# jperezrua/mfas

Hardware: AMD Instinct MI355X
Metric: candidate-archs trained/sec (NTU inner loop) (higher is better)
Workload: dtype f32

## Files before the change

### mfas_amd/csrc/launches.hip.h

```cpp
#pragma once
#include <stdint.h>
#include <vector>

struct Launch {
    int sweep_g = -1, upd = 0, fwd = 0;
    int64_t sweep_t = 0;
    int chain_g = -1;
    int64_t chain_t = 0;
    int gather_g = -1, gather_n = 0;
    int64_t gather_b = 0;
};

static void epoch_launches(int ngroups, bool same_group, int64_t T, bool gather, std::vector<Launch>& out) {
    out.clear();
    gather = gather && ngroups == 2;
    auto add = [&](int gs, int upd, int fwd, int64_t ts, int gc, int64_t tc) -> Launch& {
        out.push_back(Launch{gs, upd, fwd, ts, gc, tc});
        return out.back();
    };
    auto rows = [&](Launch& l, int g, int64_t b, int n) { if (gather) { l.gather_g = g; l.gather_b = b; l.gather_n = n; } };
    for (int g = 0; g < ngroups; ++g) rows(add(g, 0, 1, 0, -1, 0), g, 0, T > 1 ? 2 : 1);
    if (ngroups == 1 && same_group) {
        for (int64_t t = 0; t < T; ++t) add(0, 1, t + 1 < T, t, 0, t);
    } else if (ngroups == 1) {
        for (int64_t t = 0; t < T; ++t) { add(-1, 0, 0, 0, 0, t); add(0, 1, t + 1 < T, t, -1, 0); }
    } else {
        add(-1, 0, 0, 0, 0, 0);
        for (int64_t t = 0; t < T; ++t) {
            const int fwd = t + 1 < T;
            Launch& a = add(0, 1, fwd, t, 1, t);
            if (t >= 1 && t + 1 < T) rows(a, 1, t + 1, 1);
            Launch& b = add(1, 1, fwd, t, fwd ? 0 : -1, t + 1);
            if (fwd && t + 2 < T) rows(b, 0, t + 2, 1);
        }
    }
}
```

### mfas_amd/csrc/mfas_hip.hip

```cpp
#include <hip/hip_runtime.h>
#include <hip/hip_fp16.h>
#pragma clang fp contract(off)
#include <stdint.h>
#include <stdio.h>
#include <string.h>
#include <math.h>
#include <algorithm>
#include <string>
#include <vector>
#include <thread>
#include <chrono>
#include <dlfcn.h>

#include "mfas_hip.h"

#include "common.hip.h"
#include "sweep.hip.h"
#include "chain.hip.h"

struct StepArgs {
    SweepArgs sa;
    ChainArgs ca;
    int32_t nchain, _pad;
    GatherArgs ga;
};

template <int MB, bool NT, int WPE, bool LEAN, int NS = 1>
__global__ void __launch_bounds__(STEP_THREADS, WPE) k_step(const StepArgs a) {
    extern __shared__ __attribute__((aligned(16))) float lds[];
    const int bid = (int)blockIdx.x;
    if (bid < a.nchain) {
        if constexpr (NS > 1) {
            const int Kp = a.nchain / NS, part = bid / Kp, c = bid - part * Kp;
            if (c < a.ca.ncand) chain_split<NS>(a.ca, chain_step_of(a.ca), c, part, lds);
        } else
        if constexpr (LEAN) { chain_lean<MB, 0, (WPE >= 4 ? 8 : 16)>(a.ca, chain_step_of(a.ca), bid, lds, lean_pre<MB>(a.ca, bid)); chain_lean_tail<MB, 0>(a.ca, chain_step_of(a.ca), bid, lds); }
        else chain_body<MB, false>(a.ca, chain_step_of(a.ca), bid, lds);
    }
    else if (bid < a.nchain + a.ga.nblocks) gather_body(a.ga, a.ga.cands[bid - a.nchain], a.sa.g, a.sa.tab, a.sa.order, (int)threadIdx.x);
    else if (bid < a.nchain + a.ga.nblocks + a.sa.ntap) sweep_tap_body<MB, NT, SweepU<MB, WPE>::v>(a.sa, bid - a.nchain - a.ga.nblocks, lds);
    else sweep_body<MB, NT, SweepU<MB, WPE>::v>(a.sa, sweep_step_of(a.sa), bid - a.nchain - a.ga.nblocks - a.sa.ntap, lds);
}

template <int MB, bool NT, int NS = 1>
__global__ void __launch_bounds__(STEP_THREADS, 4) k_step_same(const StepArgs a) {
    extern __shared__ __attribute__((aligned(16))) float lds[];
    const int bid = (int)blockIdx.x;
    if (bid < a.nchain) {
        if constexpr (NS > 1) {
            const int Kp = a.nchain / NS, part = bid / Kp, c = bid - part * Kp;
            if (c < a.ca.ncand) chain_split<NS>(a.ca, chain_step_of(a.ca), c, part, lds);
        } else chain_body<MB, false, true>(a.ca, chain_step_of(a.ca), bid, lds);
    } else sweep_body<MB, NT, SweepU<MB, 4>::v, true>(a.sa, sweep_step_of(a.sa), bid - a.nchain, lds);
}

template <int MB, bool LEAN>
__global__ void __launch_bounds__(STEP_THREADS, 2) k_chain(const ChainArgs a) {
    extern __shared__ __attribute__((aligned(16))) float lds[];
    if constexpr (LEAN) { chain_lean<MB>(a, chain_step_of(a), (int)blockIdx.x, lds, lean_pre<MB>(a, (int)blockIdx.x)); chain_lean_tail<MB, 0>(a, chain_step_of(a), (int)blockIdx.x, lds); }
    else chain_body<MB, true>(a, chain_step_of(a), (int)blockIdx.x, lds);
}

#include "wide.hip.h"
#include "persist.hip.h"
#include "eval.hip.h"
#include "pack.hip.h"

#include "builds.hip.h"
#include "plan.hip.h"

struct LaunchRecord {
    struct Entry { BuildKey key; const void* fn; int64_t n; };
    std::vector<Entry> entries;
    void clear() { entries.clear(); }
// ... 552 lines not shown
```

### mfas_amd/csrc/plan.hip.h

```cpp
#pragma once
struct Tuning {
    int persist = -1;
    int no_lean_chain = 0;
    int groups = 0;
    int same_group = -1;
    int no_tap_major = 0;
    int force_tap_major = 0;
    int no_red_in_sweep = 0;
    double occ_bytes = -1.0;
    int no_xcd_placement = 0;
    int n_xcd = 0;
    int persist_trace = 0;
    int nt = -1;
    int eval_no_x16 = 0;
    int eval_no_msplit = 0;
    int eval_no_b3 = 0;
    int eval_no_wl = 0;
    int no_gather = 0;
    int gather_verbose = 0;
    int no_plain_chain = 0;
    int persist_verbose = 0;
    int prof_every = 16;
    int chain_split = -1;
    int test_not_resident = -1;
// ... 96 lines not shown

static Geo make_geo(const mfas_hyper* hp) {
    Geo g;
    memset(&g, 0, sizeof(g));
    g.R = hp->R; g.C = hp->C; g.Rp = ceil16(hp->R); g.Cp = ceil16(hp->C);
    g.nrb = g.Rp / 16; g.ncb = g.Cp / 16; g.B = hp->B;
    g.MB = (hp->B + 15) / 16; if (g.MB == 3) g.MB = 4;
    g.Bp = g.MB * 16;
    g.bn = hp->bn != 0; g.alphas = hp->alphas != 0; g.multitask = hp->multitask != 0;
    g.use_drop = hp->drpt > 1e-10;
    g.drop_scale = g.use_drop ? (float)(1.0 / (1.0 - hp->drpt)) : 1.0f;
    g.drop_thr = g.use_drop ? (uint32_t)floor(hp->drpt * 16777216.0) : 0u;
    g.bn_eps = (float)hp->bn_eps; g.bn_mom = (float)hp->bn_momentum;
    g.vec_cell_stride = 5 * g.Rp + 16;
    g.vec_head = MFAS_MAX_CELLS * g.vec_cell_stride;
    for (int j = 0; j < MFAS_MAX_TAPS; ++j) { g.sw[j] = ceil16(hp->s_sizes[j]); g.vw[j] = ceil16(hp->v_sizes[j]); }
    g.loss_mode = hp->loss_mode == 1 ? 1 : 0;
    g.f1_th = (float)hp->f1_threshold;
    return g;
}

static size_t res_batch_lds(const mfas_hyper* hp, const Geo& g, int cc) {
    return hp->tap_bits == 16 ? (size_t)g.Bp * (cc + 8) * 2 : (size_t)g.Bp * (cc + 4) * 4;
}
static size_t res_unit_lds(const mfas_hyper* hp, const Geo& g, int cc, int nu) {
    return (size_t)nu * 2 * res_batch_lds(hp, g, cc) + (size_t)STEP_NW * g.MB * 256 * 4 + 4 * PERSIST_LDS_WORDS + 64;
}
static size_t sweep_unit_lds(const Geo& g, const SegDesc& d) {
    const int nrb = d.rows_p / 16;
    size_t fl = (size_t)g.Bp * (d.cc + 16) + (size_t)g.Bp * (d.cc + 4) + (size_t)g.Bp * (d.rows_p + 16);
    if (nrb < STEP_NW && d.kind <= KIND_V) fl += (size_t)STEP_NW * nrb * g.MB * 256;
    return fl * 4;
}
static size_t wide_unit_lds(const SegDesc& d) {
    return wide_sweep_lds_floats(std::min(16 * WIDE_KB, d.cc), std::min(16 * WIDE_RBG, d.rows_p)) * 4;
}
static size_t wide_chain_lds(const Geo& g) { return wide_chain_lds_floats(g.Rp, g.Cp, g.Bp) * 4; }
static size_t vec_lds(const Geo& g) { return (size_t)3 * (MFAS_MAX_CELLS * g.vec_cell_stride + g.Cp) * 4; }
static size_t lean_chain_lds(const Geo& g) {
    return ((size_t)2 * MFAS_MAX_CELLS * g.Bp * 20 + (size_t)g.Bp * (g.Cp + 4) + MFAS_MAX_CELLS * 16 + 3 * g.Bp + 16
            + (size_t)(g.alphas ? 2 : 1) * MFAS_MAX_CELLS * g.MB * 256 + vec_lds(g) / 4 + LEAN_SCR + 8 + LeanLds<1>::stage_floats() + (size_t)g.Bp * 64) * 4;
}

struct ChunkPlan {
    bool want_persist = false;
    int target = 0, nu = 1;
    bool plan_res = false;
    int nfeat = 0, max_fcc = 0;
    bool res_ok = false, res_wide = false, lean_ok = false;
    int nres_wg = 0;
    bool resident = false;
};

static ChunkPlan plan_chunk(const mfas_hyper* hp, const Geo& g, const int32_t* confs, const int32_t* n_cells, int K, int chunk_cols,
                            int n_cus, bool allow_persist, const Tuning& tu) {
    ChunkPlan lp;
    lp.want_persist = allow_persist && tu.persist != 0;
    lp.lean_ok = g.nrb == 1 && g.ncb <= 4 && g.MB <= 2 && lean_chain_lds(g) <= 78 * 1024 && !tu.no_lean_chain;
    lp.plan_res = lp.want_persist && g.nrb == 1 && g.MB <= 2 && lp.lean_ok;
    auto feat_units = [&](int cc_target, int* max_cc) {
        int64_t n = 0;
        int mx = 0;
        for (int k = 0; k < K; ++k)
            for (int i = 0; i < n_cells[k] && i < MFAS_MAX_CELLS; ++i) {
                const int sw = ceil16(hp->s_sizes[confs[(k * 4 + i) * 3] & 7]), vw = ceil16(hp->v_sizes[confs[(k * 4 + i) * 3 + 1] & 7]);
                const int cs = pick_chunk(sw, cc_target), cv = pick_chunk(vw, cc_target);
// ... 49 lines not shown
}

struct GroupPlan {
    int c0 = 0, nc = 0;
    double alg_state = 0, alg_feat = 0;
    std::vector<SegDesc> descs;
    std::vector<TapDesc> taps;
};

struct LayoutPlan {
    Geo g;
    int chunk = 0;
    std::vector<CandDev> cands;
    std::vector<SegDesc> descs;
    std::vector<int> desc_start;
    std::vector<int64_t> nparams;
    std::vector<int64_t> cand_plane_base, cand_plane_size;
    int64_t plane_stride = 0, wt_size = 0, step_total = 0;
    double bytes_per_launch = 0.0;
    bool persist = false;
    bool res_chain = false;
    bool res_wide = false;
    int nres = 0;
    int res_nu = 1;
    int nres_wg = 0;
    int res_buf_words = 0;
    bool wide = false;
    std::vector<int> wide_start;
    bool lean_chain = false;
    bool same_group = false;
    int chain_split = 0;
    bool red_in_sweep = false;
    bool nontemporal = false;
    double occ_bytes = 0;
    int mbe = 4, nrbw = 1;
    bool yf_in_lds = false, vec_in_lds = false;
    size_t lds_step = 0, lds_chain = 0, lds_eval = 0;
    bool fits_lds = false;
    size_t lds_split = 0;
    size_t lds_president = 0;
    std::vector<GroupPlan> groups;
    std::vector<SegDesc> pdescs;
    std::vector<int32_t> need;
    std::vector<int32_t> role;
};

static int plan_layout_as(const mfas_hyper* hp, const int32_t* confs, const int32_t* n_cells, const uint32_t* drop_seeds, int K, int chunk_cols,
                          int n_cus, bool allow_persist, const Tuning& tu, const bool wide, LayoutPlan& pl) {
    pl = LayoutPlan();
    pl.wide = wide;
    Geo& g = pl.g;
    g = make_geo(hp);
    const int vec_size = (g.vec_head + g.Cp + 63) & ~63;

    ChunkPlan lp;
    if (wide) {
        lp.target = chunk_cols > 0 ? std::min(16 * WIDE_KB, chunk_cols) : 16 * WIDE_KB;
        lp.target = std::max(16, (lp.target / 16) * 16);
    } else {
        lp = plan_chunk(hp, g, confs, n_cells, K, chunk_cols, n_cus, allow_persist, tu);
        if (lp.res_ok && !lp.resident)
            lp = plan_chunk(hp, g, confs, n_cells, K, chunk_cols, n_cus, false, tu);
    }
    const int target = pl.chunk = lp.target;
    pl.cands.resize(K);
    pl.desc_start.assign(K + 1, 0);
// ... 285 lines not shown
            std::vector<int> prim(nwg), sec(nwg, -1);
            for (int w = 0; w < nwg; ++w) {
                prim[w] = res_cand[w];
                if (pl.res_nu == 2 && w + nwg < (int)res_cand.size()) sec[w] = res_cand[w + nwg];
            }
            for (int c = 0; c < K; ++c) {
                bool any = false;
                for (int w = 0; w < nwg; ++w) any = any || prim[w] == c;
                if (!any) continue;
                const int x = roomiest();
                if (!slots[x].empty()) { take(x, c); chain_xcd[c] = x; }
                for (int w = 0; w < nwg; ++w)
                    if (prim[w] == c && !wg_done[w] && !slots[x].empty()) { take(x, K + w); wg_done[w] = 1; }
            }
            std::vector<int> wg_xcd(nwg, -1);
            for (int b = 0; b < G; ++b) if (role[b] >= K) wg_xcd[role[b] - K] = b % NX;
            for (int c = 0; c < K; ++c) {
                if (chain_xcd[c] >= 0) continue;
                std::vector<int> votes(NX, 0);
                for (int w = 0; w < nwg; ++w) if ((prim[w] == c || sec[w] == c) && wg_xcd[w] >= 0) votes[wg_xcd[w]]++;
                int bx = -1;
                for (int x = 0; x < NX; ++x) if (!slots[x].empty() && (bx < 0 || votes[x] > votes[bx])) bx = x;
                if (bx >= 0) { take(bx, c); chain_xcd[c] = bx; }
            }
            for (int w = 0; w < nwg; ++w)
                if (!wg_done[w]) { const int x = roomiest(); take(x, K + w); wg_done[w] = 1; }
            bool ok = true;
            for (int b = 0; b < G; ++b) ok = ok && role[b] >= 0;
            if (ok) pl.role = role;
        }
    }
    pl.nontemporal = (double)pl.plane_stride * 12.0 > 200.0 * 1024 * 1024;
    if (tu.nt >= 0) pl.nontemporal = tu.nt != 0;
    return MFAS_OK;
}

static int plan_layout(const mfas_hyper* hp, const int32_t* confs, const int32_t* n_cells, const uint32_t* drop_seeds, int K, int chunk_cols,
                       int n_cus, bool allow_persist, const Tuning& tu, LayoutPlan& pl) {
    if (!batch_resident_refuses(hp)) {
        if (int rc = plan_layout_as(hp, confs, n_cells, drop_seeds, K, chunk_cols, n_cus, allow_persist, tu, false, pl)) return rc;
        if (pl.fits_lds) return MFAS_OK;
    }
    return plan_layout_as(hp, confs, n_cells, drop_seeds, K, chunk_cols, n_cus, allow_persist, tu, true, pl);
}

static PlanFacts plan_facts(const LayoutPlan& pl) {
    PlanFacts f;
    f.wide = pl.wide; f.MB = pl.g.MB; f.lean_chain = pl.lean_chain; f.same_group = pl.same_group; f.chain_split = pl.chain_split;
    f.ngroups = (int)pl.groups.size(); f.nontemporal = pl.nontemporal; f.persist = pl.persist; f.res_wide = pl.res_wide; f.res_nu = pl.res_nu;
    f.mbe = pl.mbe; f.nrbw = pl.nrbw; f.nrb = pl.g.nrb;
    return f;
}
```

### mfas_amd/csrc/sweep.hip.h

```cpp
#pragma once
template <int MB, bool NT, int SWEEP_U, bool COH = false>
__device__ __forceinline__ void tile_run(float* Wp, float* Mp, float* Vp, const int rb, const int nkb, const int kb0,
                                         const int kbs, const float* xt, const int ST, const float* xn, const int SN,
                                         const float (&dyf)[MB * 4], const float gsc, const AdamC& ac, const bool upd,
                                         const bool fwd, f32x4 (&yacc)[MB], float* T, const int tstride_rb,
                                         const int lane, const int nj) {
    const int l15 = lane & 15, lg = lane >> 4;
    const float a_ss = ac.ss, a_bc2s = ac.bc2s, a_w1 = ac.w1, a_b2 = ac.b2, a_w2 = ac.w2, a_eps = ac.eps, a_wd = ac.wd;
    for (int kbb = kb0; kbb < nkb; kbb += SWEEP_U * kbs) {
        f32x4 w4[SWEEP_U], m4[SWEEP_U], v4[SWEEP_U];
#pragma unroll
        for (int u = 0; u < SWEEP_U; ++u) {
            const int kb = kbb + u * kbs;
            if (kb < nkb) {
                const int64_t off = ((int64_t)rb * nkb + kb) * 256 + lane * 4;
                w4[u] = NT ? __builtin_nontemporal_load(reinterpret_cast<const f32x4*>(Wp + off))
                           : *reinterpret_cast<const f32x4*>(Wp + off);
                if (upd) {
                    m4[u] = NT ? __builtin_nontemporal_load(reinterpret_cast<const f32x4*>(Mp + off))
                               : *reinterpret_cast<const f32x4*>(Mp + off);
                    v4[u] = NT ? __builtin_nontemporal_load(reinterpret_cast<const f32x4*>(Vp + off))
                               : *reinterpret_cast<const f32x4*>(Vp + off);
                }
            }
        }
#pragma unroll
        for (int u = 0; u < SWEEP_U; ++u) {
            const int kb = kbb + u * kbs;
            if (kb < nkb) {
                const int64_t off = ((int64_t)rb * nkb + kb) * 256 + lane * 4;
                if (upd) {
                    f32x4 acc = {0.f, 0.f, 0.f, 0.f};
                    DW_BATCH_LOOP(MB, (COH ? MB * 4 : nj), acc = MFMA16(xt[(4 * j + lg) * ST + kb * 16 + l15], dyf[j], acc))
                    { f32x4 w = w4[u], m = m4[u], v = v4[u];
                      adam4(w, m, v, acc * gsc, a_ss, a_bc2s, a_w1, a_b2, a_w2, a_eps, a_wd);
                      w4[u] = w; m4[u] = m; v4[u] = v; }
                    if (NT) {
                        __builtin_nontemporal_store(w4[u], reinterpret_cast<f32x4*>(Wp + off));
                        __builtin_nontemporal_store(m4[u], reinterpret_cast<f32x4*>(Mp + off));
                        __builtin_nontemporal_store(v4[u], reinterpret_cast<f32x4*>(Vp + off));
                    } else {
                        *reinterpret_cast<f32x4*>(Wp + off) = w4[u];
                        *reinterpret_cast<f32x4*>(Mp + off) = m4[u];
                        *reinterpret_cast<f32x4*>(Vp + off) = v4[u];
                    }
                    if (T) {
                        float* Tt = T + ((int64_t)kb * tstride_rb + rb) * 256;
                        const int base = (((l15 >> 2) * 16 + 4 * lg) << 2) + (l15 & 3);
#pragma unroll
                        for (int q = 0; q < 4; ++q) Tt[base + 4 * q] = w4[u][q];
                    }
                }
                if (fwd) {
#pragma unroll
                    for (int mb = 0; mb < MB; ++mb) {
                        const f32x4 x4 = *reinterpret_cast<const f32x4*>(xn + (mb * 16 + l15) * SN + kb * 16 + 4 * lg);
#pragma unroll
                        for (int q = 0; q < 4; ++q) yacc[mb] = MFMA16(x4[q], w4[u][q], yacc[mb]);
                    }
                }
            }
        }
    }
}

#define STEP_NW 8
#define STEP_THREADS (STEP_NW * 64)

struct SweepArgs {
    const SegDesc* desc;
    const TapDesc* tdesc;
    int32_t ntap, _padt;
    const CandDev* cands;
    float* plane;
    int64_t plane_stride;
    float* wt;
    float* stepbuf;
    mfas_table tab;
    const int32_t* order;
    int64_t pos_t, pos_n;
    int32_t base_t, base_n, nvalid_t, nvalid_n;
    int32_t do_update, do_forward;
    AdamC ac;
    Geo g;
    uint32_t* red_cnt;
    const uint32_t* cellflag;
    uint32_t flag_target;
    int32_t* flag_status;
    const char* gather;
    int64_t g_cand_stride, g_par_stride;
    int32_t g_par_t, g_par_n;
};

__device__ __forceinline__ int64_t gather_tap_off(const Geo& g, const int kind, const int tap, const int eb) {
    int64_t o = 0;
#pragma unroll
    for (int u = 0; u < MFAS_MAX_TAPS; ++u) {
        if (kind == KIND_V || u < tap) o += g.sw[u];
        if (kind == KIND_V && u < tap) o += g.vw[u];
    }
    return o * g.Bp * eb;
}

struct GatherArgs {
    const CandDev* cands;
    char* buf;
    int64_t cand_stride, par_stride;
    int64_t pos[2];
    int32_t base[2], nvalid[2], par[2];
    int32_t nsets, nblocks;
};

__device__ __forceinline__ void gather_body(const GatherArgs& ga, const CandDev& cd, const Geo& g, const mfas_table& tab,
                                            const int32_t* order, const int tid) {
    const int eb = tab.dtype == MFAS_DT_F32 ? 4 : 2;
    const int32_t* ordp = cand_order(order, g, cd.gidx);
    uint32_t used = 0;
    for (int i = 0; i < cd.L; ++i) used |= (1u << cd.conf[i][0]) | (1u << (MFAS_MAX_TAPS + cd.conf[i][1]));
#pragma unroll
    for (int s = 0; s < 2; ++s) {
        if (s >= ga.nsets) break;
        char* dst0 = ga.buf + (int64_t)cd.gidx * ga.cand_stride + (int64_t)ga.par[s] * ga.par_stride;
        for (int kt = 0; kt < 2 * MFAS_MAX_TAPS; ++kt) {
            if (!((used >> kt) & 1u)) continue;
// ... 19 lines not shown
                    if (e < nvec) {
                        const int b = e / vpr, c = e - b * vpr;
                        *reinterpret_cast<u32x4*>(dst + ((int64_t)b * w) * eb + ((int64_t)c << 4)) = v[u];
                    }
                }
            }
        }
    }
}

struct SweepStep {
    int64_t pos_t, pos_n;
    int32_t base_t, base_n, nvalid_t, nvalid_n;
    int32_t upd, fwd;
    float ss, bc2s;
};
__device__ __forceinline__ SweepStep sweep_step_of(const SweepArgs& a) {
    SweepStep s;
    s.pos_t = a.pos_t; s.pos_n = a.pos_n; s.base_t = a.base_t; s.base_n = a.base_n;
    s.nvalid_t = a.nvalid_t; s.nvalid_n = a.nvalid_n; s.upd = a.do_update; s.fwd = a.do_forward;
    s.ss = a.ac.ss; s.bc2s = a.ac.bc2s;
    return s;
}


#ifdef MFAS_CHAIN_TIMING
#define SW_UNIT_STAMP(k) do { if (COH && a.cellflag && a.flag_target == 16u && threadIdx.x == 0 && d.cell == 0 && d.kind == KIND_S && d.k0 == 0 && d.cand == 0) a.flag_status[64 + 29 + (k)] = (int32_t)wall_clock64(); } while (0)
#define SW_END_STAMP() do { if (COH && a.cellflag && a.flag_target == 16u && threadIdx.x == 0) { atomicMax(reinterpret_cast<uint32_t*>(&a.flag_status[64 + 27]), (uint32_t)wall_clock64()); \
        atomicMax(reinterpret_cast<uint32_t*>(&a.flag_status[128 + d.cell * 4 + d.kind]), (uint32_t)wall_clock64()); } } while (0)
#else
#define SW_END_STAMP() do { } while (0)
#define SW_UNIT_STAMP(k) do { } while (0)
#endif
template <int MB, bool NT, int U, bool COH = false>
__device__ __forceinline__ void sweep_body(const SweepArgs& a, const SweepStep& st, const int bid, float* lds) {
    const SegDesc d = a.desc[bid];
    const CandDev& cd = a.cands[d.cand];
    const int tid = threadIdx.x, lane = tid & 63, wave = tid >> 6;
    const int l15 = lane & 15, lg = lane >> 4;
    constexpr int Bp = MB * 16;
    const int cc = d.cc, rows_p = d.rows_p, nrb = rows_p >> 4, nkb = cc >> 4;
    const int ST = cc + 16;
    const int SN = cc + 4;
    const int SD = rows_p + 16;
    float* xt = lds;
    float* xn = xt + Bp * ST;
    float* dyl = xn + Bp * SN;
    float* wred = dyl + Bp * SD;
    const bool feat = d.kind <= KIND_V;
    const bool upd = st.upd != 0;
    const bool fwd = (st.fwd != 0) && feat;
    if (!upd && !fwd) return;
    const int64_t sbo = cd.step_off;
    const bool red = a.red_cnt != nullptr;

    if (!COH && a.gather && feat) {
        const char* gb = a.gather + (int64_t)cd.gidx * a.g_cand_stride + gather_tap_off(a.g, d.kind, d.tap, a.tab.dtype == MFAS_DT_F32 ? 4 : 2);
        if (upd) stage_table(xt, ST, gb + (int64_t)a.g_par_t * a.g_par_stride, a.tab.dtype, d.width, d.k0, cc, nullptr, 0, 0, st.nvalid_t, Bp, tid, STEP_THREADS);
        if (fwd) stage_table(xn, SN, gb + (int64_t)a.g_par_n * a.g_par_stride, a.tab.dtype, d.width, d.k0, cc, nullptr, 0, 0, st.nvalid_n, Bp, tid, STEP_THREADS);
    } else {
    if (upd && feat) {
        const void* tp = d.kind == KIND_S ? a.tab.s[d.tap] : a.tab.v[d.tap];
        stage_table(xt, ST, tp, a.tab.dtype, d.width, d.k0, cc, cand_order(a.order, a.g, cd.gidx), st.pos_t, st.base_t, st.nvalid_t, Bp, tid, STEP_THREADS);
    }
    if (fwd) {
        const void* tp = d.kind == KIND_S ? a.tab.s[d.tap] : a.tab.v[d.tap];
        stage_table(xn, SN, tp, a.tab.dtype, d.width, d.k0, cc, cand_order(a.order, a.g, cd.gidx), st.pos_n, st.base_n, st.nvalid_n, Bp, tid, STEP_THREADS);
    }
    }
    if constexpr (COH) {
        if (upd && a.cellflag) {
            __shared__ int s_go;
            if (tid == 0) {
                const int slot = d.kind == KIND_HEAD ? cd.L - 1 : (d.kind == KIND_OUT ? d.cell - 1 : d.cell);
                const uint32_t* f = a.cellflag + (size_t)cd.gidx * CELLFLAG_STRIDE + slot;
                uint32_t spins = 0;
                int go = 1;
                while (ld_u32_relaxed(f) < a.flag_target) {
                    __builtin_amdgcn_s_sleep(2);
                    if (++spins > CELLFLAG_SPIN_LIMIT) { go = 0; atomicMax(&a.flag_status[cd.gidx], 2); break; }
                }
                s_go = go;
#ifdef MFAS_CHAIN_TIMING
                if (a.flag_target == 16u && slot == 0 && d.kind <= KIND_V) atomicMin(reinterpret_cast<uint32_t*>(&a.flag_status[64 + 28]), (uint32_t)wall_clock64());
#endif
            }
            __syncthreads();
            if (!s_go) return;
            SW_UNIT_STAMP(0);
        }
    }
    if (upd) {
        if (!feat) {
            const int xcell = d.kind == KIND_OUT ? d.cell - 1 : cd.L - 1;
            stage_f32<COH>(xt, ST, a.stepbuf, sbo + a.g.sb_xo + (int64_t)xcell * Bp * a.g.Rp + d.k0, a.g.Rp, cc, Bp, tid, STEP_THREADS);
        }
        const int64_t dsrc = d.kind == KIND_HEAD ? sbo + a.g.sb_dlog : sbo + a.g.sb_dy + (int64_t)d.cell * Bp * a.g.Rp;
        stage_f32<COH>(dyl, SD, a.stepbuf, dsrc + d.rb0 * 16, d.seg_nrb * 16, rows_p, Bp, tid, STEP_THREADS);
    }
    __syncthreads();
    SW_UNIT_STAMP(1);

    float* Wp = a.plane + d.w_off;
    float* Mp = Wp + a.plane_stride;
    float* Vp = Mp + a.plane_stride;
    const AdamC ac = adam_consts(a.ac, upd ? st.ss : 0.f, upd ? st.bc2s : 1.f);
    float gsc = 1.0f;
    if (a.g.alphas && feat && upd) gsc = ldc1<COH>(a.stepbuf + sbo + a.g.sb_gsc + d.cell * 2 + d.kind);

    const bool split_k = nrb < STEP_NW;
    const int rb0 = split_k ? 0 : wave, rbs = split_k ? 1 : STEP_NW;
    const int kb0 = split_k ? wave : 0, kbs = split_k ? STEP_NW : 1;
    const int64_t part = sbo + a.g.sb_part + (((int64_t)(cd.part_cell_off[d.cell] + d.part_idx) * d.seg_nrb * MB) << 8) +
                         (((int64_t)d.rb0 * MB) << 8);

    for (int rb = rb0; rb < nrb; rb += rbs) {
        float dyf[MB * 4];
#pragma unroll
        for (int j = 0; j < MB * 4; ++j) dyf[j] = upd ? dyl[(4 * j + lg) * SD + rb * 16 + l15] : 0.f;
        f32x4 yacc[MB];
#pragma unroll
        for (int mb = 0; mb < MB; ++mb) yacc[mb] = (f32x4){0.f, 0.f, 0.f, 0.f};
        tile_run<MB, NT, U, COH>(Wp, Mp, Vp, rb, nkb, kb0, kbs, xt, ST, xn, SN, dyf, gsc, ac, upd, fwd, yacc,
                                 d.wt_off >= 0 ? a.wt + d.wt_off + ((int64_t)(d.k0 >> 4) * d.seg_nrb + d.rb0) * 256 : nullptr, d.seg_nrb, lane, (a.g.B + 3) >> 2);
        if (fwd) {
#pragma unroll
            for (int mb = 0; mb < MB; ++mb) {
                if (split_k)
                    *reinterpret_cast<f32x4*>(wred + (((wave * nrb + rb) * MB + mb) << 8) + lane * 4) = yacc[mb];
                else if (red) stc4<true>(a.stepbuf, part + ((rb * MB + mb) << 8) + lane * 4, yacc[mb]);
                else
                    stc4<COH>(a.stepbuf, part + ((rb * MB + mb) << 8) + lane * 4, yacc[mb]);
            }
        }
    }
    SW_UNIT_STAMP(2);
    if (!fwd) { SW_END_STAMP(); return; }
    if (split_k) {
        __syncthreads();
        for (int e = tid; e < nrb * MB * 64; e += STEP_THREADS) {
            const int slot = e >> 6, ln = e & 63;
            f32x4 s = *reinterpret_cast<const f32x4*>(wred + (slot << 8) + ln * 4);
#pragma unroll
            for (int w = 1; w < STEP_NW; ++w)
                s += *reinterpret_cast<const f32x4*>(wred + ((w * nrb * MB + slot) << 8) + ln * 4);
            if (red) stc4<true>(a.stepbuf, part + (slot << 8) + ln * 4, s);
            else stc4<COH>(a.stepbuf, part + (slot << 8) + ln * 4, s);
        }
    }
    if (!red) { SW_END_STAMP(); return; }
    asm volatile("s_waitcnt vmcnt(0)" ::: "memory");
    __syncthreads();
    SW_UNIT_STAMP(3);
    int* flagw = reinterpret_cast<int*>(lds);
    const int ns_c = cd.nch_s[d.cell], nch_c = ns_c + cd.nch_v[d.cell];
    if (tid == 0) {
        uint32_t* cnt = a.red_cnt + d.cand * MFAS_MAX_CELLS + d.cell;
        const uint32_t old = __hip_atomic_fetch_add(cnt, 1u, __ATOMIC_RELAXED, __HIP_MEMORY_SCOPE_AGENT);
        const int last = old == (uint32_t)(nch_c - 1);
        if (last) __hip_atomic_store(cnt, 0u, __ATOMIC_RELAXED, __HIP_MEMORY_SCOPE_AGENT);
        flagw[0] = last;
    }
    __syncthreads();
    SW_UNIT_STAMP(4);
    if (!flagw[0]) { SW_END_STAMP(); return; }
    {
        const int snrb = d.seg_nrb;
        const int per_cell = snrb * MB * 64;
        const int64_t part0 = sbo + a.g.sb_part + (((int64_t)cd.part_cell_off[d.cell] * snrb * MB) << 8);
        const int64_t yf0 = sbo + a.g.sb_yf + (int64_t)d.cell * per_cell * 4;
        const int64_t vplane = (int64_t)MFAS_MAX_CELLS * snrb * MB * 256;
        for (int it = tid; it < per_cell; it += STEP_THREADS) {
            f32x4 accS = {0.f, 0.f, 0.f, 0.f}, accV = {0.f, 0.f, 0.f, 0.f};
            constexpr int PB = 8;
            for (int ch0 = 0; ch0 < nch_c; ch0 += PB) {
                f32x4 p8[PB];
#pragma unroll
                for (int u = 0; u < PB; ++u)
// ... 66 lines not shown
```

### mfas_amd/csrc/train.hip.h

```cpp
#pragma once
struct TrainCall {
    mfas_population* p = nullptr;
    const mfas_table *train = nullptr, *dev = nullptr;
    const int32_t* order = nullptr; const float* step_scalars = nullptr;
    int epochs = 0, first = 0, last = 0, B = 0;
    bool segment = false, resume = false, do_dev = false, snapshot_best = false;
    int64_t max_steps = -1, N = 0, nb = 0;
    AdamC ac; StepArgs st;
    std::vector<Launch> launches;
    int64_t launches_T = -1;
    int64_t split_launches[2] = {0, 0};
    size_t ev_used = 0;
    std::vector<double> ev_bytes; int64_t nlaunch = 0;
    bool use_gather = false;
    int64_t g_par_stride = 0, g_cand_stride = 0;
    std::vector<uint32_t> aborts;
    std::vector<double> best_acc;
    double metric_scale = 1.0; std::vector<DevStats> hstats;
    int elt() const { return train->dtype == MFAS_DT_F32 ? 4 : 2; }
    double dev_metric(int k, int ep) const { return (double)hstats[(size_t)k * epochs + ep].dev_corr * metric_scale / (double)dev->N; }
};

static void base_args(mfas_population* p, const mfas_table& tab, const int32_t* order, const Geo& g, const AdamC& ac, SweepArgs& sa, ChainArgs& ca) {
    const LayoutPlan& pl = p->plan;
    sa.cands = p->d_cands; sa.plane = p->plane; sa.plane_stride = pl.plane_stride; sa.wt = p->wt;
    sa.stepbuf = p->stepbuf; sa.tab = tab; sa.order = order; sa.g = g; sa.ac = ac;
    ca.plane = p->plane; ca.plane_stride = pl.plane_stride; ca.wt = p->wt; ca.stepbuf = p->stepbuf;
    ca.tab = tab; ca.order = order; ca.g = g; ca.status = p->d_status; ca.ac = ac;
    ca.yf_in_lds = pl.yf_in_lds ? 1 : 0; ca.vec_in_lds = pl.vec_in_lds ? 1 : 0; ca.pos_w = p->d_posw;
}

static hipError_t setup_gather(TrainCall& c) {
    mfas_population* p = c.p;
    const Geo& g = c.st.sa.g;
    c.use_gather = p->plan.groups.size() == 2 && !p->plan.persist && c.order && g.order_stride > 0 && !p->tune.no_gather;
    if (!c.use_gather) return hipSuccess;
    int64_t totw = 0;
    for (int u = 0; u < MFAS_MAX_TAPS; ++u) totw += g.sw[u] + g.vw[u];
    c.g_par_stride = totw * g.Bp * c.elt(); c.g_cand_stride = 2 * c.g_par_stride;
    const size_t need = (size_t)c.g_cand_stride * p->K;
    if (p->gather_cap < need) {
        hipFree(p->d_gather); p->d_gather = nullptr; p->gather_cap = 0;
        hipError_t e = hipMalloc(&p->d_gather, need);
        if (e != hipSuccess) { c.use_gather = false; (void)hipGetLastError(); return hipSuccess; }
        p->gather_cap = need;
    }
    if (p->tune.gather_verbose) fprintf(stderr, "[gather] on: %d candidates, %.1f MB of gathered rows\n", p->K, (double)need / 1e6);
    return hipSuccess;
}

static hipError_t init_args(TrainCall& c, int64_t ep) {
    mfas_population* p = c.p; StepArgs& st = c.st;
    const LayoutPlan& pl = p->plan; const int K = p->K;
    c.launches_T = -1;
    Geo g = pl.g;
    g.order_stride = (p->hp.order_per_candidate && c.order) ? (int64_t)c.epochs * c.N : 0;
    memset(&st, 0, sizeof(st));
    base_args(p, *c.train, c.order, g, c.ac, st.sa, st.ca);
    st.ca.E = c.epochs; st.ca.stats = p->d_stats;
    st.sa.red_cnt = pl.red_in_sweep ? p->d_red_cnt : nullptr; st.ca.yf_reduced = pl.red_in_sweep ? 1 : 0;
    hipError_t e_ = hipSuccess;
    if (pl.red_in_sweep) e_ = hipMemsetAsync(p->d_red_cnt, 0, sizeof(uint32_t) * K * MFAS_MAX_CELLS, p->stream);
    if (e_ == hipSuccess && pl.same_group) e_ = hipMemsetAsync(p->d_cellflag, 0, sizeof(uint32_t) * K * CELLFLAG_STRIDE, p->stream);
    if (e_ == hipSuccess && pl.chain_split) e_ = hipMemsetAsync(p->d_xch, 0xFF, sizeof(float) * (size_t)K * XCH_CAND_FLOATS, p->stream);
    st.ca.xch = p->d_xch; st.ca.nsplit = pl.chain_split; st.ca.xpar = 0;
    c.split_launches[0] = c.split_launches[1] = 0;
    if (e_ == hipSuccess && ep > 0 && pl.same_group && pl.chain_split)
        e_ = hipMemsetD32Async(reinterpret_cast<hipDeviceptr_t>(p->d_cellflag), (int)((uint32_t)pl.chain_split * (uint32_t)(ep * c.nb)),
                               (size_t)K * CELLFLAG_STRIDE, p->stream);
    return e_ != hipSuccess ? e_ : setup_gather(c);
}

struct ProfBracket {
    TrainCall& c;
    const bool on;
    const double bytes;
    ProfBracket(TrainCall& c_, bool on_, double bytes_) : c(c_), on(on_), bytes(bytes_) {
        if (!on) return;
        mfas_population* p = c.p;
        if (p->ev.size() < c.ev_used + 2) {
            hipEvent_t e0, e1;
            hipEventCreate(&e0); hipEventCreate(&e1); p->ev.push_back(e0); p->ev.push_back(e1);
        }
        hipEventRecord(p->ev[c.ev_used], p->stream);
    }
    ~ProfBracket() {
        if (!on) return;
        hipEventRecord(c.p->ev[c.ev_used + 1], c.p->stream);
        c.ev_used += 2; c.ev_bytes.push_back(bytes);
    }
};

static void launch_record(TrainCall& c, int64_t ep, const Launch& L) {
    mfas_population* p = c.p;
    const LayoutPlan& pl = p->plan;
    StepArgs& st = c.st;
    const int64_t N = c.N;
    const int B = c.B, gs = L.sweep_g, gc = L.chain_g;
    auto nvalid = [&](int64_t t) { return (int)std::min<int64_t>(B, N - t * B); };
    unsigned nsw = 0, nch = 0;
    st.ga.nblocks = 0; st.ga.nsets = 0; st.sa.gather = nullptr;
    if (c.use_gather) {
        GatherArgs& ga = st.ga;
        ga.buf = p->d_gather; ga.cand_stride = c.g_cand_stride; ga.par_stride = c.g_par_stride;
        for (int s = 0; s < L.gather_n; ++s) {
            const int64_t t = L.gather_b + s;
            ga.pos[s] = ep * N + t * B; ga.base[s] = (int)(t * B); ga.nvalid[s] = nvalid(t); ga.par[s] = (int)(t & 1);
        }
        if (L.gather_g >= 0) { ga.nsets = L.gather_n; ga.cands = p->d_cands + pl.groups[L.gather_g].c0; ga.nblocks = pl.groups[L.gather_g].nc; }
        if (gs >= 0 && L.upd) {
            st.sa.gather = p->d_gather; st.sa.g_cand_stride = c.g_cand_stride; st.sa.g_par_stride = c.g_par_stride;
            st.sa.g_par_t = (int)(L.sweep_t & 1); st.sa.g_par_n = (int)((L.sweep_t + 1) & 1);
        }
    }
    if (gs >= 0) {
        SweepArgs& s = st.sa;
        const int64_t ts = L.sweep_t, tn = L.fwd && L.upd ? ts + 1 : ts, gstep = ep * c.nb + ts;
        s.desc = p->groups[gs].d_descs;
        s.tdesc = p->groups[gs].d_taps; s.ntap = (int)pl.groups[gs].taps.size();
        s.do_update = L.upd; s.do_forward = L.fwd;
        s.pos_t = ep * N + ts * B; s.base_t = (int)(ts * B); s.nvalid_t = nvalid(ts);
        s.pos_n = ep * N + tn * B; s.base_n = (int)(tn * B); s.nvalid_n = nvalid(tn);
        s.ac.ss = L.upd ? c.step_scalars[2 * gstep] : 0.f;
        s.ac.bc2s = L.upd ? c.step_scalars[2 * gstep + 1] : 1.f;
        nsw = (unsigned)(pl.groups[gs].descs.size() + pl.groups[gs].taps.size());
    } else st.sa.ntap = 0;
    if (gc >= 0) {
        ChainArgs& ca = st.ca;
        const int64_t tc = L.chain_t, gstep = ep * c.nb + tc;
        ca.cands = p->d_cands + pl.groups[gc].c0;
        ca.pos_t = ep * N + tc * B; ca.base_t = (int)(tc * B); ca.nvalid = nvalid(tc);
        ca.gstep = (int)gstep; ca.epoch = (int)ep;
        ca.ac.ss = c.step_scalars[2 * gstep]; ca.ac.bc2s = c.step_scalars[2 * gstep + 1];
        nch = (unsigned)pl.groups[gc].nc;
    }
    st.nchain = (int)nch;
    if (nsw == 0) {
        launch_build(p, chain_build(chain_key(plan_facts(pl))), nch, pl.lds_chain, p->stream, st.ca);
        return;
    }
    ProfBracket prof(c, p->profiling && L.upd && L.fwd && ((c.nlaunch++ % p->prof_every) == 0),
                     pl.groups[gs].alg_state + pl.groups[gs].alg_feat * c.elt() + 8.0 * B * pl.groups[gs].nc);
    const bool same = pl.same_group && gc == gs && L.upd, split = pl.chain_split && nch > 0;
    if (split) {
        st.ca.ncand = (int)nch; st.ca.xpar = (int)(c.split_launches[gc & 1]++ & 1);
        st.nchain = pl.chain_split * (int)((nch + 7) & ~7u);
    }
    if (same) {
        st.sa.cellflag = p->d_cellflag; st.ca.cellflag = p->d_cellflag;
        st.sa.flag_target = st.ca.flag_target = (split ? (uint32_t)pl.chain_split : 1u) * ((uint32_t)st.ca.gstep + 1u);
        st.sa.flag_status = p->d_status;
    }
    const BuildKey key = step_key(plan_facts(pl), nch, same, pl.groups[gs].alg_state > pl.occ_bytes);
    launch_build(p, step_build(key), (unsigned)st.nchain + st.ga.nblocks + nsw, split ? pl.lds_split : pl.lds_step, p->stream, st);
    if (same) { st.sa.cellflag = nullptr; st.ca.cellflag = nullptr; }
}

static hipError_t persist_epoch_once(TrainCall& c, int ep, int64_t T) {
    mfas_population* p = c.p;
    const LayoutPlan& pl = p->plan;
    const Geo& g = pl.g;
    const int K = p->K;
    if (p->tune.test_not_resident >= 0 && ep >= p->tune.test_not_resident) { c.aborts[ep] = PERSIST_ABORT_NOT_RESIDENT; return hipSuccess; }
    hipError_t e = hipMemsetAsync(p->d_sync, 0, sizeof(uint32_t) * ((size_t)K * PERSIST_SYNC_STRIDE + 64), p->stream);
    if (e != hipSuccess) return e;
    PersistArgs pa;
    memset(&pa, 0, sizeof(pa));
    pa.sa = c.st.sa; pa.ca = c.st.ca;
    pa.sa.desc = p->d_pdescs; pa.sa.tdesc = nullptr; pa.sa.ntap = 0;
    pa.ca.cands = p->d_cands;
    pa.nchain = K; pa.nitems = (int)pl.pdescs.size(); pa.nres = pl.nres; pa.res_chain = pl.res_chain ? 1 : 0; pa.res_wide = pl.res_wide ? 1 : 0;
    pa.res_nu = pl.res_nu; pa.nres_wg = pl.nres_wg; pa.res_buf_words = pl.res_buf_words;
    pa.T = (int)T; pa.epoch = ep;
    pa.lose_step = p->tune.test_lose_step;
// ... 137 lines not shown
    c.ac.eps = (float)hp.adam_eps; c.ac.wd = (float)hp.wd; c.ac.ss = 0.f; c.ac.bc2s = 1.f;
    c.aborts.assign(epochs, 0u);
    HIPCHK(init_args(c, c.first));
    p->prof_launches = 0; p->prof_ms = 0.0; p->prof_bytes = 0.0;
    if (p->plan.persist) {
        const int64_t steps = (int64_t)epochs * c.nb;
        if (p->scal_cap < (size_t)steps * 2) {
            hipFree(p->d_scal); p->d_scal = nullptr;
            HIPCHK(hipMalloc(&p->d_scal, sizeof(float) * steps * 2));
            p->scal_cap = (size_t)steps * 2;
        }
        const size_t have = (size_t)(c.max_steps >= 0 ? std::min<int64_t>(c.max_steps, steps) : steps) * 2;
        HIPCHK(hipMemcpyAsync(p->d_scal, c.step_scalars, sizeof(float) * have, hipMemcpyHostToDevice, p->stream));
    }
    return MFAS_OK;
}

static int train_epoch(TrainCall& c, int ep, int64_t T) {
    mfas_population* p = c.p;
    if (p->plan.persist) {
        HIPCHK(persist_epoch(c, ep, T));
        if (c.aborts[ep] == PERSIST_ABORT_NOT_RESIDENT) {
            if (p->tune.persist_verbose) fprintf(stderr, "[persist] epoch %d: the resident grid never became resident; falling back to launch-per-phase\n", ep);
            if (int rc = persist_fallback(p)) return rc;
            HIPCHK(init_args(c, ep));
            c.aborts[ep] = 0;
        } else if (c.aborts[ep]) {
            HIPCHK(hipStreamSynchronize(p->stream));
            return fail(MFAS_EHIP, "persistent step loop: a workgroup timed out waiting for its dependency (abort code 1: the epoch was "
                                   "abandoned half way, this population's parameters are not usable)");
        }
    }
    if (!p->plan.persist) {
        if (c.launches_T != T) { epoch_launches((int)p->plan.groups.size(), p->plan.same_group, T, c.use_gather, c.launches); c.launches_T = T; }
        for (const Launch& L : c.launches) launch_record(c, ep, L);
    }
    HIPCHK(hipGetLastError());
    return MFAS_OK;
}

static int train_dev(TrainCall& c, int ep) {
    mfas_population* p = c.p;
    const int K = p->K;
    EvalArgs ea;
    memset(&ea, 0, sizeof(ea));
    ea.cands = p->d_cands; ea.plane = p->plane; ea.tab = *c.dev; ea.row0 = 0; ea.nrows = c.dev->N;
    ea.cand0 = 0; ea.epoch = ep; ea.E = c.epochs; ea.g = c.st.sa.g; ea.stats = p->d_stats; ea.pos_w = p->d_posw;
    HIPCHK(launch_eval(p, ea, K, p->stream));
    if (!c.snapshot_best) return MFAS_OK;
    HIPCHK(hipMemcpyAsync(c.hstats.data(), p->d_stats, sizeof(DevStats) * K * c.epochs, hipMemcpyDeviceToHost, p->stream));
    HIPCHK(hipStreamSynchronize(p->stream));
    for (int k = 0; k < K; ++k) {
        const double acc = c.dev_metric(k, ep);
        if (acc > c.best_acc[k]) {
            c.best_acc[k] = acc;
            HIPCHK(hipMemcpyAsync(p->best + p->plan.cand_plane_base[k], p->plane + p->plan.cand_plane_base[k],
                                  sizeof(float) * p->plan.cand_plane_size[k], hipMemcpyDeviceToDevice, p->stream));
        }
    }
    return MFAS_OK;
}

static int train_end(TrainCall& c, mfas_epoch_stats* stats, int32_t* status) {
    mfas_population* p = c.p;
    const int K = p->K, epochs = c.epochs;
    if (c.snapshot_best && c.do_dev && c.last == epochs) {
        HIPCHK(hipMemcpyAsync(p->plane, p->best, sizeof(float) * (size_t)p->plan.plane_stride, hipMemcpyDeviceToDevice, p->stream));
// ... 108 lines not shown
```

Measured before the change: 34.09.

## Defer feature-segment W/m/v stores to every second step via paired Adam updates

Pairs consecutive update launches per group. The first (virtual) launch computes Adam in registers but skips writing W/m/v back to memory. The second (double) launch recomputes the previous step's gradient from a retained previous-batch dy area and gathered rows, applies both Adam steps, and stores once. This is meant to halve weight/optimizer-state write traffic for streaming feature segments. In exchange it triples the gather row sets, alternates between two dy areas in the step buffer, enlarges LDS per unit, and redoes the previous step's MFMA work.

```diff
diff --git a/mfas_amd/csrc/launches.hip.h b/mfas_amd/csrc/launches.hip.h
--- a/mfas_amd/csrc/launches.hip.h
+++ b/mfas_amd/csrc/launches.hip.h
@@ -9,6 +9,7 @@
     int64_t chain_t = 0;
     int gather_g = -1, gather_n = 0;
     int64_t gather_b = 0;
+    int mode = 0;
 };
 
 static void epoch_launches(int ngroups, bool same_group, int64_t T, bool gather, std::vector<Launch>& out) {
@@ -35,3 +36,24 @@
         }
     }
 }
+
+enum { LAUNCH_PLAIN = 0, LAUNCH_VIRTUAL = 1, LAUNCH_DOUBLE = 2 };
+
+static inline void mark_deferred(int ngroups, bool same_group, std::vector<Launch>& list) {
+    for (Launch& l : list) l.mode = LAUNCH_PLAIN;
+    if (ngroups != 2 || same_group) return;
+    for (int g = 0; g < 2; ++g) {
+        Launch* open = nullptr;
+        int64_t n = 0;
+        for (Launch& l : list) {
+            if (l.sweep_g != g || !l.upd) continue;
+            if (open) { open->mode = LAUNCH_VIRTUAL; l.mode = LAUNCH_DOUBLE; open = nullptr; }
+            else if (n >= g) open = &l;
+            ++n;
+        }
+    }
+}
+
+static inline int row_sets(bool deferring) { return deferring ? 3 : 2; }
+static inline int row_set_of(int64_t batch, bool deferring) { return (int)(batch % row_sets(deferring)); }
+static inline int dy_area_of(int64_t step, bool deferring) { return deferring ? (int)(step & 1) : 0; }
diff --git a/mfas_amd/csrc/mfas_hip.hip b/mfas_amd/csrc/mfas_hip.hip
--- a/mfas_amd/csrc/mfas_hip.hip
+++ b/mfas_amd/csrc/mfas_hip.hip
@@ -39,7 +39,7 @@
     }
     else if (bid < a.nchain + a.ga.nblocks) gather_body(a.ga, a.ga.cands[bid - a.nchain], a.sa.g, a.sa.tab, a.sa.order, (int)threadIdx.x);
     else if (bid < a.nchain + a.ga.nblocks + a.sa.ntap) sweep_tap_body<MB, NT, SweepU<MB, WPE>::v>(a.sa, bid - a.nchain - a.ga.nblocks, lds);
-    else sweep_body<MB, NT, SweepU<MB, WPE>::v>(a.sa, sweep_step_of(a.sa), bid - a.nchain - a.ga.nblocks - a.sa.ntap, lds);
+    else sweep_body<MB, NT, SweepU<MB, WPE>::v, false, !LEAN>(a.sa, sweep_step_of(a.sa), bid - a.nchain - a.ga.nblocks - a.sa.ntap, lds);
 }
 
 template <int MB, bool NT, int NS = 1>
diff --git a/mfas_amd/csrc/plan.hip.h b/mfas_amd/csrc/plan.hip.h
--- a/mfas_amd/csrc/plan.hip.h
+++ b/mfas_amd/csrc/plan.hip.h
@@ -152,6 +152,13 @@
     if (nrb < STEP_NW && d.kind <= KIND_V) fl += (size_t)STEP_NW * nrb * g.MB * 256;
     return fl * 4;
 }
+static size_t sweep_unit_lds_double(const Geo& g, const SegDesc& d) {
+    const int nrb = d.rows_p / 16;
+    const size_t replay = (size_t)g.Bp * (d.cc + 16) + (size_t)g.Bp * (d.rows_p + 16), slab = (size_t)STEP_NW * g.MB * 256;
+    size_t fl = (size_t)g.Bp * (d.cc + 16) + (size_t)g.Bp * (d.cc + 4) + (size_t)g.Bp * (d.rows_p + 16);
+    fl += nrb < STEP_NW ? (size_t)(nrb - 1) * slab + std::max(slab, replay) : replay;
+    return fl * 4;
+}
 static size_t wide_unit_lds(const SegDesc& d) {
     return wide_sweep_lds_floats(std::min(16 * WIDE_KB, d.cc), std::min(16 * WIDE_RBG, d.rows_p)) * 4;
 }
@@ -267,6 +274,8 @@
     int chain_split = 0;
     bool red_in_sweep = false;
     bool nontemporal = false;
+    bool defer = false;
+    int64_t sb_dy_alt = 0;
     double occ_bytes = 0;
     int mbe = 4, nrbw = 1;
     bool yf_in_lds = false, vec_in_lds = false;
@@ -618,6 +627,18 @@
     }
     pl.nontemporal = (double)pl.plane_stride * 12.0 > 200.0 * 1024 * 1024;
     if (tu.nt >= 0) pl.nontemporal = tu.nt != 0;
+    pl.defer = pl.groups.size() == 2 && !wide && !pl.persist && !pl.same_group && !pl.lean_chain && !g.alphas;
+    for (const GroupPlan& gr : pl.groups) {
+        if (!gr.taps.empty()) pl.defer = false;
+        for (const SegDesc& d : gr.descs)
+            if (d.kind <= KIND_V && sweep_unit_lds_double(g, d) > pl.lds_step) pl.defer = false;
+    }
+    if (pl.defer) {
+        pl.sb_dy_alt = g.sb_size;
+        g.sb_size = (g.sb_size + (int64_t)MFAS_MAX_CELLS * g.Bp * g.Rp + 63) & ~63LL;
+        for (int k = 0; k < K; ++k) pl.cands[k].step_off = (int64_t)k * g.sb_size;
+        pl.step_total = (int64_t)K * g.sb_size;
+    }
     return MFAS_OK;
 }
 
diff --git a/mfas_amd/csrc/sweep.hip.h b/mfas_amd/csrc/sweep.hip.h
--- a/mfas_amd/csrc/sweep.hip.h
+++ b/mfas_amd/csrc/sweep.hip.h
@@ -1,10 +1,14 @@
 #pragma once
-template <int MB, bool NT, int SWEEP_U, bool COH = false>
+#include "launches.hip.h"
+template <int MB, bool NT, int SWEEP_U, bool COH = false, bool DBL = false>
 __device__ __forceinline__ void tile_run(float* Wp, float* Mp, float* Vp, const int rb, const int nkb, const int kb0,
                                          const int kbs, const float* xt, const int ST, const float* xn, const int SN,
                                          const float (&dyf)[MB * 4], const float gsc, const AdamC& ac, const bool upd,
                                          const bool fwd, f32x4 (&yacc)[MB], float* T, const int tstride_rb,
-                                         const int lane, const int nj) {
+                                         const int lane, const int nj, const bool store = true, const float* xp = nullptr,
+                                         const float* dyp = nullptr, const float* dyc = nullptr, const int SDp = 0,
+                                         const float ss_p = 0.f, const float bc2s_p = 1.f) {
+    static_assert(!(DBL && COH), "the same-group launch defers nothing");
     const int l15 = lane & 15, lg = lane >> 4;
     const float a_ss = ac.ss, a_bc2s = ac.bc2s, a_w1 = ac.w1, a_b2 = ac.b2, a_w2 = ac.w2, a_eps = ac.eps, a_wd = ac.wd;
     for (int kbb = kb0; kbb < nkb; kbb += SWEEP_U * kbs) {
@@ -30,12 +34,24 @@
             if (kb < nkb) {
                 const int64_t off = ((int64_t)rb * nkb + kb) * 256 + lane * 4;
                 if (upd) {
+                    int dq = lg * SDp + rb * 16 + l15;
+                    if constexpr (DBL) asm volatile("" : "+v"(dq));
+                    if constexpr (DBL) {
+                        f32x4 accp = {0.f, 0.f, 0.f, 0.f};
+                        DW_BATCH_LOOP(MB, nj, accp = MFMA16(xp[(4 * j + lg) * ST + kb * 16 + l15], dyp[dq + 4 * j * SDp], accp))
+                        f32x4 w = w4[u], m = m4[u], v = v4[u];
+                        adam4(w, m, v, accp * gsc, ss_p, bc2s_p, a_w1, a_b2, a_w2, a_eps, a_wd);
+                        w4[u] = w; m4[u] = m; v4[u] = v;
+                        __builtin_amdgcn_sched_barrier(0);
+                    }
                     f32x4 acc = {0.f, 0.f, 0.f, 0.f};
-                    DW_BATCH_LOOP(MB, (COH ? MB * 4 : nj), acc = MFMA16(xt[(4 * j + lg) * ST + kb * 16 + l15], dyf[j], acc))
+                    if constexpr (DBL) { DW_BATCH_LOOP(MB, nj, acc = MFMA16(xt[(4 * j + lg) * ST + kb * 16 + l15], dyc[dq + 4 * j * SDp], acc)) }
+                    else { DW_BATCH_LOOP(MB, (COH ? MB * 4 : nj), acc = MFMA16(xt[(4 * j + lg) * ST + kb * 16 + l15], dyf[j], acc)) }
                     { f32x4 w = w4[u], m = m4[u], v = v4[u];
                       adam4(w, m, v, acc * gsc, a_ss, a_bc2s, a_w1, a_b2, a_w2, a_eps, a_wd);
                       w4[u] = w; m4[u] = m; v4[u] = v; }
-                    if (NT) {
+                    if (!COH && !DBL && !store) {
+                    } else if (NT) {
                         __builtin_nontemporal_store(w4[u], reinterpret_cast<f32x4*>(Wp + off));
                         __builtin_nontemporal_store(m4[u], reinterpret_cast<f32x4*>(Mp + off));
                         __builtin_nontemporal_store(v4[u], reinterpret_cast<f32x4*>(Vp + off));
@@ -90,6 +106,10 @@
     const char* gather;
     int64_t g_cand_stride, g_par_stride;
     int32_t g_par_t, g_par_n;
+    int32_t mode, g_par_p;
+    int64_t pos_p, sb_dy_prev;
+    int32_t base_p, nvalid_p;
+    float ss_p, bc2s_p;
 };
 
 __device__ __forceinline__ int64_t gather_tap_off(const Geo& g, const int kind, const int tap, const int eb) {
@@ -175,7 +195,7 @@
 #define SW_END_STAMP() do { } while (0)
 #define SW_UNIT_STAMP(k) do { } while (0)
 #endif
-template <int MB, bool NT, int U, bool COH = false>
+template <int MB, bool NT, int U, bool COH = false, bool DEFER = !COH>
 __device__ __forceinline__ void sweep_body(const SweepArgs& a, const SweepStep& st, const int bid, float* lds) {
     const SegDesc d = a.desc[bid];
     const CandDev& cd = a.cands[d.cand];
@@ -189,21 +209,28 @@
     float* xt = lds;
     float* xn = xt + Bp * ST;
     float* dyl = xn + Bp * SN;
-    float* wred = dyl + Bp * SD;
     const bool feat = d.kind <= KIND_V;
     const bool upd = st.upd != 0;
     const bool fwd = (st.fwd != 0) && feat;
     if (!upd && !fwd) return;
+    float* wred = dyl + Bp * SD;
+    const bool split_k = nrb < STEP_NW;
+    const int mode = (DEFER && feat && upd) ? a.mode : LAUNCH_PLAIN;
+    const bool dbl = mode == LAUNCH_DOUBLE;
+    float* xp = wred + (split_k ? (nrb - 1) * STEP_NW * MB * 256 : 0);
+    float* dyp = xp + Bp * ST;
     const int64_t sbo = cd.step_off;
     const bool red = a.red_cnt != nullptr;
 
     if (!COH && a.gather && feat) {
         const char* gb = a.gather + (int64_t)cd.gidx * a.g_cand_stride + gather_tap_off(a.g, d.kind, d.tap, a.tab.dtype == MFAS_DT_F32 ? 4 : 2);
+        if (dbl) stage_table(xp, ST, gb + (int64_t)a.g_par_p * a.g_par_stride, a.tab.dtype, d.width, d.k0, cc, nullptr, 0, 0, a.nvalid_p, Bp, tid, STEP_THREADS);
         if (upd) stage_table(xt, ST, gb + (int64_t)a.g_par_t * a.g_par_stride, a.tab.dtype, d.width, d.k0, cc, nullptr, 0, 0, st.nvalid_t, Bp, tid, STEP_THREADS);
         if (fwd) stage_table(xn, SN, gb + (int64_t)a.g_par_n * a.g_par_stride, a.tab.dtype, d.width, d.k0, cc, nullptr, 0, 0, st.nvalid_n, Bp, tid, STEP_THREADS);
     } else {
     if (upd && feat) {
         const void* tp = d.kind == KIND_S ? a.tab.s[d.tap] : a.tab.v[d.tap];
+        if (dbl) stage_table(xp, ST, tp, a.tab.dtype, d.width, d.k0, cc, cand_order(a.order, a.g, cd.gidx), a.pos_p, a.base_p, a.nvalid_p, Bp, tid, STEP_THREADS);
         stage_table(xt, ST, tp, a.tab.dtype, d.width, d.k0, cc, cand_order(a.order, a.g, cd.gidx), st.pos_t, st.base_t, st.nvalid_t, Bp, tid, STEP_THREADS);
     }
     if (fwd) {
@@ -240,6 +267,7 @@
         }
         const int64_t dsrc = d.kind == KIND_HEAD ? sbo + a.g.sb_dlog : sbo + a.g.sb_dy + (int64_t)d.cell * Bp * a.g.Rp;
         stage_f32<COH>(dyl, SD, a.stepbuf, dsrc + d.rb0 * 16, d.seg_nrb * 16, rows_p, Bp, tid, STEP_THREADS);
+        if (dbl) stage_f32<false>(dyp, SD, a.stepbuf, sbo + a.sb_dy_prev + (int64_t)d.cell * Bp * a.g.Rp + d.rb0 * 16, d.seg_nrb * 16, rows_p, Bp, tid, STEP_THREADS);
     }
     __syncthreads();
     SW_UNIT_STAMP(1);
@@ -251,7 +279,6 @@
     float gsc = 1.0f;
     if (a.g.alphas && feat && upd) gsc = ldc1<COH>(a.stepbuf + sbo + a.g.sb_gsc + d.cell * 2 + d.kind);
 
-    const bool split_k = nrb < STEP_NW;
     const int rb0 = split_k ? 0 : wave, rbs = split_k ? 1 : STEP_NW;
     const int kb0 = split_k ? wave : 0, kbs = split_k ? STEP_NW : 1;
     const int64_t part = sbo + a.g.sb_part + (((int64_t)(cd.part_cell_off[d.cell] + d.part_idx) * d.seg_nrb * MB) << 8) +
@@ -259,18 +286,30 @@
 
     for (int rb = rb0; rb < nrb; rb += rbs) {
         float dyf[MB * 4];
-#pragma unroll
-        for (int j = 0; j < MB * 4; ++j) dyf[j] = upd ? dyl[(4 * j + lg) * SD + rb * 16 + l15] : 0.f;
         f32x4 yacc[MB];
 #pragma unroll
         for (int mb = 0; mb < MB; ++mb) yacc[mb] = (f32x4){0.f, 0.f, 0.f, 0.f};
-        tile_run<MB, NT, U, COH>(Wp, Mp, Vp, rb, nkb, kb0, kbs, xt, ST, xn, SN, dyf, gsc, ac, upd, fwd, yacc,
-                                 d.wt_off >= 0 ? a.wt + d.wt_off + ((int64_t)(d.k0 >> 4) * d.seg_nrb + d.rb0) * 256 : nullptr, d.seg_nrb, lane, (a.g.B + 3) >> 2);
+        float* Tt = d.wt_off >= 0 ? a.wt + d.wt_off + ((int64_t)(d.k0 >> 4) * d.seg_nrb + d.rb0) * 256 : nullptr;
+        bool plain_walk = true;
+        if constexpr (DEFER) {
+            if (dbl) {
+                plain_walk = false;
+                tile_run<MB, NT, (U > 1 ? U / 2 : 1), false, true>(Wp, Mp, Vp, rb, nkb, kb0, kbs, xt, ST, xn, SN, dyf, gsc, ac, upd, fwd, yacc, Tt, d.seg_nrb,
+                                                                    lane, (a.g.B + 3) >> 2, true, xp, dyp, dyl, SD, a.ss_p, a.bc2s_p);
+                if (split_k && fwd && rb == nrb - 1) __syncthreads();
+            }
+        }
+        if (plain_walk) {
+#pragma unroll
+            for (int j = 0; j < MB * 4; ++j) dyf[j] = upd ? dyl[(4 * j + lg) * SD + rb * 16 + l15] : 0.f;
+            tile_run<MB, NT, U, COH>(Wp, Mp, Vp, rb, nkb, kb0, kbs, xt, ST, xn, SN, dyf, gsc, ac, upd, fwd, yacc, Tt, d.seg_nrb, lane,
+                                     (a.g.B + 3) >> 2, mode != LAUNCH_VIRTUAL);
+        }
         if (fwd) {
 #pragma unroll
             for (int mb = 0; mb < MB; ++mb) {
                 if (split_k)
-                    *reinterpret_cast<f32x4*>(wred + (((wave * nrb + rb) * MB + mb) << 8) + lane * 4) = yacc[mb];
+                    *reinterpret_cast<f32x4*>(wred + (((rb * STEP_NW + wave) * MB + mb) << 8) + lane * 4) = yacc[mb];
                 else if (red) stc4<true>(a.stepbuf, part + ((rb * MB + mb) << 8) + lane * 4, yacc[mb]);
                 else
                     stc4<COH>(a.stepbuf, part + ((rb * MB + mb) << 8) + lane * 4, yacc[mb]);
@@ -283,10 +322,11 @@
         __syncthreads();
         for (int e = tid; e < nrb * MB * 64; e += STEP_THREADS) {
             const int slot = e >> 6, ln = e & 63;
-            f32x4 s = *reinterpret_cast<const f32x4*>(wred + (slot << 8) + ln * 4);
+            const int srb = slot / MB, smb = slot - srb * MB;
+            f32x4 s = *reinterpret_cast<const f32x4*>(wred + (((srb * STEP_NW) * MB + smb) << 8) + ln * 4);
 #pragma unroll
             for (int w = 1; w < STEP_NW; ++w)
-                s += *reinterpret_cast<const f32x4*>(wred + ((w * nrb * MB + slot) << 8) + ln * 4);
+                s += *reinterpret_cast<const f32x4*>(wred + (((srb * STEP_NW + w) * MB + smb) << 8) + ln * 4);
             if (red) stc4<true>(a.stepbuf, part + (slot << 8) + ln * 4, s);
             else stc4<COH>(a.stepbuf, part + (slot << 8) + ln * 4, s);
         }
diff --git a/mfas_amd/csrc/train.hip.h b/mfas_amd/csrc/train.hip.h
--- a/mfas_amd/csrc/train.hip.h
+++ b/mfas_amd/csrc/train.hip.h
@@ -37,7 +37,7 @@
     if (!c.use_gather) return hipSuccess;
     int64_t totw = 0;
     for (int u = 0; u < MFAS_MAX_TAPS; ++u) totw += g.sw[u] + g.vw[u];
-    c.g_par_stride = totw * g.Bp * c.elt(); c.g_cand_stride = 2 * c.g_par_stride;
+    c.g_par_stride = totw * g.Bp * c.elt(); c.g_cand_stride = row_sets(p->plan.defer) * c.g_par_stride;
     const size_t need = (size_t)c.g_cand_stride * p->K;
     if (p->gather_cap < need) {
         hipFree(p->d_gather); p->d_gather = nullptr; p->gather_cap = 0;
@@ -45,7 +45,9 @@
         if (e != hipSuccess) { c.use_gather = false; (void)hipGetLastError(); return hipSuccess; }
         p->gather_cap = need;
     }
-    if (p->tune.gather_verbose) fprintf(stderr, "[gather] on: %d candidates, %.1f MB of gathered rows\n", p->K, (double)need / 1e6);
+    if (p->tune.gather_verbose)
+        fprintf(stderr, "[gather] on: %d candidates, %.1f MB of gathered rows, %d row sets%s\n", p->K, (double)need / 1e6, row_sets(p->plan.defer),
+                p->plan.defer ? " (feature segments store W / m / v every second step)" : "");
     return hipSuccess;
 }
 
@@ -105,12 +107,13 @@
         ga.buf = p->d_gather; ga.cand_stride = c.g_cand_stride; ga.par_stride = c.g_par_stride;
         for (int s = 0; s < L.gather_n; ++s) {
             const int64_t t = L.gather_b + s;
-            ga.pos[s] = ep * N + t * B; ga.base[s] = (int)(t * B); ga.nvalid[s] = nvalid(t); ga.par[s] = (int)(t & 1);
+            ga.pos[s] = ep * N + t * B; ga.base[s] = (int)(t * B); ga.nvalid[s] = nvalid(t); ga.par[s] = row_set_of(t, pl.defer);
         }
         if (L.gather_g >= 0) { ga.nsets = L.gather_n; ga.cands = p->d_cands + pl.groups[L.gather_g].c0; ga.nblocks = pl.groups[L.gather_g].nc; }
         if (gs >= 0 && L.upd) {
             st.sa.gather = p->d_gather; st.sa.g_cand_stride = c.g_cand_stride; st.sa.g_par_stride = c.g_par_stride;
-            st.sa.g_par_t = (int)(L.sweep_t & 1); st.sa.g_par_n = (int)((L.sweep_t + 1) & 1);
+            st.sa.g_par_t = row_set_of(L.sweep_t, pl.defer); st.sa.g_par_n = row_set_of(L.sweep_t + 1, pl.defer);
+            st.sa.g_par_p = row_set_of(std::max<int64_t>(L.sweep_t - 1, 0), pl.defer);
         }
     }
     if (gs >= 0) {
@@ -123,6 +126,13 @@
         s.pos_n = ep * N + tn * B; s.base_n = (int)(tn * B); s.nvalid_n = nvalid(tn);
         s.ac.ss = L.upd ? c.step_scalars[2 * gstep] : 0.f;
         s.ac.bc2s = L.upd ? c.step_scalars[2 * gstep + 1] : 1.f;
+        s.mode = L.mode;
+        s.g.sb_dy = dy_area_of(ts, pl.defer) ? pl.sb_dy_alt : pl.g.sb_dy;
+        if (L.mode == LAUNCH_DOUBLE) {
+            s.pos_p = ep * N + (ts - 1) * B; s.base_p = (int)((ts - 1) * B); s.nvalid_p = nvalid(ts - 1);
+            s.sb_dy_prev = dy_area_of(ts - 1, pl.defer) ? pl.sb_dy_alt : pl.g.sb_dy;
+            s.ss_p = c.step_scalars[2 * (gstep - 1)]; s.bc2s_p = c.step_scalars[2 * (gstep - 1) + 1];
+        }
         nsw = (unsigned)(pl.groups[gs].descs.size() + pl.groups[gs].taps.size());
     } else st.sa.ntap = 0;
     if (gc >= 0) {
@@ -132,6 +142,7 @@
         ca.pos_t = ep * N + tc * B; ca.base_t = (int)(tc * B); ca.nvalid = nvalid(tc);
         ca.gstep = (int)gstep; ca.epoch = (int)ep;
         ca.ac.ss = c.step_scalars[2 * gstep]; ca.ac.bc2s = c.step_scalars[2 * gstep + 1];
+        ca.g.sb_dy = dy_area_of(tc, pl.defer) ? pl.sb_dy_alt : pl.g.sb_dy;
         nch = (unsigned)pl.groups[gc].nc;
     }
     st.nchain = (int)nch;
@@ -139,7 +150,12 @@
         launch_build(p, chain_build(chain_key(plan_facts(pl))), nch, pl.lds_chain, p->stream, st.ca);
         return;
     }
-    ProfBracket prof(c, p->profiling && L.upd && L.fwd && ((c.nlaunch++ % p->prof_every) == 0),
+    bool sampled = false;
+    if (p->profiling && L.upd && L.fwd) {
+        const int64_t n = c.nlaunch++, pe = p->prof_every;
+        sampled = n % pe == (((n / pe) & 1) ? 2 % pe : 0);
+    }
+    ProfBracket prof(c, sampled,
                      pl.groups[gs].alg_state + pl.groups[gs].alg_feat * c.elt() + 8.0 * B * pl.groups[gs].nc);
     const bool same = pl.same_group && gc == gs && L.upd, split = pl.chain_split && nch > 0;
     if (split) {
@@ -343,7 +359,11 @@
         }
     }
     if (!p->plan.persist) {
-        if (c.launches_T != T) { epoch_launches((int)p->plan.groups.size(), p->plan.same_group, T, c.use_gather, c.launches); c.launches_T = T; }
+        if (c.launches_T != T) {
+            epoch_launches((int)p->plan.groups.size(), p->plan.same_group, T, c.use_gather, c.launches);
+            if (p->plan.defer) mark_deferred((int)p->plan.groups.size(), p->plan.same_group, c.launches);
+            c.launches_T = T;
+        }
         for (const Launch& L : c.launches) launch_record(c, ep, L);
     }
     HIPCHK(hipGetLastError());
```

Result: faster. 36.32 (median of 6 runs) (+6.5%).
